# sehyun03/MulActSeg

Measured on AMD Instinct MI355X. Metric: superpixels scored/sec, higher is better.
Workload: dtype f32; 1 GPU; acquisition-round: PixBal+ban-ignore scorer on resident logits, Cityscapes pool shape [4,20,1024,2048] per step; per rank K single-pass scans (class prior + region sums + histograms) of its shard, then exchange 1 (all-gather class sums) + device class weights (k_class_weight) + weighted finalize + ban + exchange 2 (all-gather scores) + replicated K4 (keys, radix sort, fair-counting budget walk) ov; nseg=2048, id_dtype=int64, regions_scored=679936, budget_clicks=11159, regions_selected=6688

## Files before the change

### include/mulactseg_hip.h

```cpp
#ifndef MULACTSEG_HIP_H
#define MULACTSEG_HIP_H

#include <stddef.h>
#include <stdint.h>

#ifdef __cplusplus
extern "C" {
#endif

#define MAS_ID_I64 0
#define MAS_ID_I32 1
#define MAS_ID_U16 2
#define MAS_MAP_U8 3

#define MAS_MAX_CLASSES 32

#define MAS_SCORE_FRAC_BITS 40
#define MAS_PROB_FRAC_BITS 23
#define MAS_LOSS_FRAC_BITS 32

#define MAS_ABI_VERSION 9
int mas_abi_version(void);
const char* mas_error_string(int code);

// ... 62 lines not shown
                               const void* work, const float* grad, const float* weights, int N, int C, int H, int W, int S, float invT,
                               int flags, float* dz, int64_t* dzq_fix, void* stream);


int mas_region_keys(const float* score, const uint8_t* valid, const int32_t* img_rank, int64_t n_img, int S,
                    uint64_t* keys , void* stream);

size_t mas_select_workspace_bytes(int64_t n);

int mas_sort_keys_desc(const uint64_t* keys_in, int64_t n, uint64_t* keys_out, void* workspace, size_t ws_bytes,
                       void* stream);

int mas_budget_walk(const uint64_t* sorted_keys, int64_t n, const uint8_t* region_cost, const int32_t* img_of_rank,
                    int S, int64_t budget, int64_t max_out, int64_t* n_selected,
                    int32_t* sel_img, int32_t* sel_id, float* sel_score, void* workspace, size_t ws_bytes, void* stream);

int mas_region_reweight(float* score, const int32_t* dominant, int64_t n, int ban_class, const float* cls_w ,
                        void* stream);

int mas_dominant_hist(const int32_t* dominant, int64_t n, int C, uint64_t* counts , void* stream);

int mas_minmax_normalize(float* scores, int64_t n, uint32_t* scratch2, void* stream);


#define MAS_LABELS_BAD_VALUE 1

int mas_region_label_counts(const void* spx, int spx_dtype, const uint8_t* labels, int H, int W, int nseg, int num_classes, int trim_k,
                            int32_t* full , int32_t* trimmed , int32_t* status ,
                            void* stream);

// ... 204 lines not shown
```

### mulactseg_amd/_lib.py

```python
import ctypes
import os

_HERE = os.path.dirname(os.path.abspath(__file__))
LIB_PATH = os.environ.get("MAS_LIB") or os.path.join(_HERE, "libmulactseg_hip.so")

ID_I64, ID_I32, ID_U16 = 0, 1, 2
MAP_U8 = 3
MAX_CLASSES = 32
LABELS_BAD_VALUE = 1
SCORE_FRAC, PROB_FRAC, LOSS_FRAC = 40, 23, 32
LOSS_CE, LOSS_GROUP, LOSS_GROUP_ONLY_MULTI, LOSS_DECOMP, LOSS_TCE = 1, 2, 4, 8, 16
ACC_WORDS = 8
GRAD_FRAC = 44
MS_MAX_SOURCES = 16

SK_DMA, SK_NOSPLIT = 1, 2
LOWRES_GENERIC = 1
ABI_VERSION = 9

_c = ctypes
_vp, _i, _f, _i64, _d = _c.c_void_p, _c.c_int, _c.c_float, _c.c_int64, _c.c_double


class SkOpts(ctypes.Structure):
    _fields_ = [("flags", _c.c_uint), ("spin_limit", _c.c_uint), ("stamps", _c.c_void_p)]


SIGNATURES = {
    "mas_abi_version": (_i, []),
    "mas_error_string": (_c.c_char_p, [_i]),
    "mas_class_prob_sum": (_i, [_vp, _i, _i, _i, _i, _f, _vp, _vp]),
    "mas_bvsb_region_accum": (_i, [_vp, _vp, _i, _vp, _i, _i, _i, _i, _i, _f, _vp, _vp, _vp]),
    "mas_region_finalize": (_i, [_vp, _vp, _i64, _i, _i, _vp, _vp, _vp, _vp, _vp]),
    "mas_region_keys": (_i, [_vp, _vp, _vp, _i64, _i, _vp, _vp]),
    "mas_select_workspace_bytes": (_c.c_size_t, [_i64]),
    "mas_sort_keys_desc": (_i, [_vp, _i64, _vp, _vp, _c.c_size_t, _vp]),
    "mas_budget_walk": (_i, [_vp, _i64, _vp, _vp, _i, _i64, _i64, _vp, _vp, _vp, _vp, _vp, _c.c_size_t, _vp]),
    "mas_region_reweight": (_i, [_vp, _vp, _i64, _i, _vp, _vp]),
    "mas_dominant_hist": (_i, [_vp, _i64, _i, _vp, _vp]),
    "mas_minmax_normalize": (_i, [_vp, _i64, _vp, _vp]),
    "mas_region_label_counts": (_i, [_vp, _i, _vp, _i, _i, _i, _i, _i, _vp, _vp, _vp, _vp]),
    "mas_region_multi_hot": (_i, [_vp, _vp, _vp, _i, _i, _vp, _vp, _vp]),
    "mas_region_dominant": (_i, [_vp, _vp, _vp, _i, _i, _i, _vp, _vp]),
    "mas_region_paint": (_i, [_vp, _i, _vp, _i, _i, _i, _vp, _i, _vp, _vp]),
    "mas_spx_max_onehot": (_i, [_vp, _i, _vp, _i, _i, _i, _i, _i, _vp, _vp, _vp, _vp, _vp]),
    "mas_iou_counts": (_i, [_vp, _vp, _vp, _i64, _i, _i64, _vp, _vp]),
    "mas_logits_iou_counts": (_i, [_vp, _vp, _i, _i, _i, _i, _i, _i64, _vp, _vp]),
    "mas_lowres_iou_counts": (_i, [_vp, _vp, _i, _i, _i, _i, _i, _i, _i, _i64, _vp, _vp]),
    "mas_single_pass_accum": (_i, [_vp, _vp, _i, _i, _i, _i, _i, _i, _f, _vp, _vp, _vp, _vp]),
    "mas_single_pass_accum_lowres": (_i, [_vp, _i, _i, _vp, _i, _i, _i, _i, _i, _i, _f, _vp, _vp, _vp, _vp]),
    "mas_single_pass_accum_lowres_opt": (_i, [_vp, _i, _i, _vp, _i, _i, _i, _i, _i, _i, _f, _vp, _vp, _vp, _c.c_uint, _vp]),
    "mas_class_weight": (_i, [_vp, _i, _i, _i64, _i, _i, _d, _vp, _vp, _vp, _vp]),
# ... 141 lines not shown
```

### mulactseg_amd/active_selection/engine.py

```python
import numpy as np
import torch


class ShardPlan:

    def __init__(self, n_img, batch_size, rank=0, world=1):
        self.n_img, self.batch_size, self.rank, self.world = n_img, batch_size, rank, world
        self.n_batches = (n_img + batch_size - 1) // batch_size
        per = (self.n_batches + world - 1) // world
        self.batch_lo = min(rank * per, self.n_batches)
        self.batch_hi = min((rank + 1) * per, self.n_batches)
        self.img_lo = min(self.batch_lo * batch_size, n_img)
        self.img_hi = min(self.batch_hi * batch_size, n_img)
        self.per_rank_imgs = per * batch_size
        self.batch_of = (np.arange(n_img) // batch_size).astype(np.int32)

    @property
    def local_indices(self):
        return list(range(self.img_lo, self.img_hi))

    @property
    def n_local(self):
        return self.img_hi - self.img_lo

# ... 74 lines not shown
        w31 = None if cls_w is None else getattr(cls_w, '_mas_w31', None)
        if w31 is None:
            w = torch.ones(hist.shape[-1], dtype=torch.float32, device=hist.device) if cls_w is None else cls_w.detach().to(hist.device)
            w31 = (w.double() * 2147483648.0).floor().to(torch.int64).view(torch.int32)[::2].contiguous()
        return self.ops.region_finalize_weighted(class_sum, hist, w31, ban_class, want_hist_i64)

    def minmax_normalize_(self, scores):
        return self.ops.minmax_normalize_(scores)

    def region_reweight_(self, scores, dominant, ban_class, cls_w):
        return self.ops.region_reweight_(scores, dominant, ban_class, cls_w)

    def dominant_hist(self, dominant, C):
        return self.ops.dominant_hist(dominant, C)

    def select(self, scores, valid, img_rank, img_of_rank, region_cost, budget, max_out):
        keys = self.ops.region_keys(scores, valid, img_rank)
        skeys = self.ops.sort_keys_desc(keys)
        nsel, simg, sid, ssc = self.ops.budget_walk(skeys, region_cost, img_of_rank, scores.shape[1], budget, max_out)
        n = int(nsel.item())
        return n, simg[:n].cpu().numpy(), sid[:n].cpu().numpy(), ssc[:n].cpu().numpy()

    def local_head(self, plan, scores, valid, img_rank, max_out):
        lo, hi = plan.img_lo, plan.img_hi
        head = torch.zeros(max_out, dtype=torch.int64, device=scores.device)
        if hi > lo:
            keys = self.ops.region_keys(scores[lo:hi].contiguous(), None if valid is None else valid[lo:hi].contiguous(),
                                        img_rank[lo:hi].contiguous())
            m = min(keys.numel(), max_out)
            head[:m] = self.ops.sort_keys_desc(keys)[:m]
        return head

    def walk_heads(self, heads, region_cost, img_of_rank, S, budget, max_out):
        nsel, simg, sid, ssc = self.ops.budget_walk(self.ops.sort_keys_desc(heads), region_cost, img_of_rank, S, budget, max_out)
        n = int(nsel.item())
        return n, simg[:n].cpu().numpy(), sid[:n].cpu().numpy(), ssc[:n].cpu().numpy()

    def select_sharded(self, plan, scores, valid, img_rank, img_of_rank, region_cost, budget, max_out):
        head = self.local_head(plan, scores, valid, img_rank, max_out)
        merged = torch.empty(plan.world * max_out, dtype=torch.int64, device=scores.device)
        _dist().all_gather_into_tensor(merged, head)
        return self.walk_heads(merged, region_cost, img_of_rank, scores.shape[1], budget, max_out)


def default_backend(device):
    return HipBackend(device)


def select_regions(backend, plan, scores, valid, img_rank, img_of_rank, region_cost, budget, max_out):
    if plan.world > 1 and max_out is not None and _dist() is not None and hasattr(backend, 'select_sharded'):
        return backend.select_sharded(plan, scores, valid, img_rank, img_of_rank, region_cost, budget, max_out)
# ... 105 lines not shown
```

### mulactseg_amd/csrc/select.hip

```cpp
#include <cstring>

#include <rocprim/device/device_radix_sort.hpp>
#include <rocprim/device/device_scan.hpp>

#include "common.h"

namespace {

constexpr int kThreads = 256;

__device__ __forceinline__ unsigned order_bits(float f) {
    const unsigned b = mas_f2u(f);
    return (b & 0x80000000u) ? ~b : (b | 0x80000000u);
}
__device__ __forceinline__ float unorder_bits(unsigned o) {
    return mas_u2f((o & 0x80000000u) ? (o & 0x7fffffffu) : ~o);
}

inline int id_bits_for(int S) {
    int b = 1;
    while ((1LL << b) < S) ++b;
    return b;
}

__global__ __launch_bounds__(kThreads) void k_region_keys(const float* __restrict__ score, const unsigned char* __restrict__ valid,
                                                           const int* __restrict__ img_rank, long long n, int S, int id_bits,
                                                           mas_u64* __restrict__ keys) {
    const long long i = (long long)blockIdx.x * kThreads + threadIdx.x;
    if (i >= n) return;
    const long long img = i / S;
    const int id = (int)(i - img * S);
    mas_u64 k = 0;
    if (!valid || valid[i]) {
        const unsigned lo = ((unsigned)img_rank[img] << id_bits) | (unsigned)id;
        k = ((mas_u64)order_bits(score[i]) << 32) | lo;
    }
    keys[i] = k;
}

__global__ __launch_bounds__(kThreads) void k_walk_cost(const mas_u64* __restrict__ keys, long long n,
                                                         const unsigned char* __restrict__ region_cost,
                                                         const int* __restrict__ img_of_rank, int S, int id_bits,
                                                         unsigned* __restrict__ cost) {
    const long long i = (long long)blockIdx.x * kThreads + threadIdx.x;
    if (i >= n) return;
    const mas_u64 k = keys[i];
    unsigned c = 0;
    if (k) {
        c = 1;
        if (region_cost) {
            const unsigned lo = (unsigned)k;
            const int id = (int)(lo & ((1u << id_bits) - 1u));
            const int img = img_of_rank[lo >> id_bits];
            c = (unsigned)region_cost[(long long)img * S + id];
        }
    }
    cost[i] = c;
}

__global__ __launch_bounds__(kThreads) void k_walk_find(const mas_u64* __restrict__ keys, const unsigned* __restrict__ prefix,
                                                         long long n, unsigned long long budget,
                                                         unsigned long long* __restrict__ n_selected) {
    const long long i = (long long)blockIdx.x * kThreads + threadIdx.x;
    if (i >= n) return;
    const bool valid = keys[i] != 0;
    const bool prev_valid = (i == 0) ? true : (keys[i - 1] != 0);
    const bool crossed = valid && (unsigned long long)prefix[i] > budget;
    const bool prev_crossed = (i > 0) && ((unsigned long long)prefix[i - 1] > budget);
    if (crossed && !prev_crossed) atomicMin(n_selected, (unsigned long long)(i + 1));
    if (!valid && prev_valid) atomicMin(n_selected, (unsigned long long)i);
    if (i == n - 1 && valid) atomicMin(n_selected, (unsigned long long)n);
}

__global__ __launch_bounds__(kThreads) void k_walk_emit(const mas_u64* __restrict__ keys, const unsigned long long* __restrict__ n_selected,
                                                         long long max_out, const int* __restrict__ img_of_rank, int id_bits,
                                                         int* __restrict__ sel_img, int* __restrict__ sel_id,
                                                         float* __restrict__ sel_score) {
    const long long i = (long long)blockIdx.x * kThreads + threadIdx.x;
    if (i >= max_out) return;
    int img = -1, id = -1;
    float s = 0.0f;
    if ((unsigned long long)i < *n_selected) {
        const mas_u64 k = keys[i];
        const unsigned lo = (unsigned)k;
        id = (int)(lo & ((1u << id_bits) - 1u));
        img = img_of_rank[lo >> id_bits];
        s = unorder_bits((unsigned)(k >> 32));
    }
    sel_img[i] = img;
    sel_id[i] = id;
    sel_score[i] = s;
}

__global__ void k_set_u64(unsigned long long* p, unsigned long long v) { *p = v; }

__global__ __launch_bounds__(kThreads) void k_region_reweight(float* __restrict__ score, const int* __restrict__ dominant,
                                                               long long n, int ban_class, const float* __restrict__ cls_w) {
    const long long i = (long long)blockIdx.x * kThreads + threadIdx.x;
    if (i >= n) return;
    const int d = dominant[i];
    float s = score[i];
    if (d == ban_class) s = 0.0f;
// ... 60 lines not shown
}

}

extern "C" size_t mas_select_workspace_bytes(int64_t n) {
    if (n <= 0) return 0;
    const size_t t = sort_temp_bytes(n), u = scan_temp_bytes(n);
    return align_up(t > u ? t : u) + 2 * align_up(sizeof(unsigned) * (size_t)n) + 256;
}

extern "C" int mas_region_keys(const float* score, const uint8_t* valid, const int32_t* img_rank, int64_t n_img, int S,
                               uint64_t* keys, void* stream) {
    if (!score || !img_rank || !keys) return MAS_ERR_NULL;
    if (n_img <= 0 || S <= 0) return MAS_ERR_SHAPE;
    const int b = id_bits_for(S);
    if (b > 24 || n_img > (1LL << (32 - b))) return MAS_ERR_RANGE;
    const long long n = (long long)n_img * S;
    const long long nblk = (n + kThreads - 1) / kThreads;
    if (nblk > 0x7fffffffLL) return MAS_ERR_SHAPE;
    hipLaunchKernelGGL(k_region_keys, dim3((unsigned)nblk), dim3(kThreads), 0, static_cast<hipStream_t>(stream), score, valid,
                       img_rank, n, S, b, reinterpret_cast<mas_u64*>(keys));
    return mas_launch_status();
}

extern "C" int mas_sort_keys_desc(const uint64_t* keys_in, int64_t n, uint64_t* keys_out, void* workspace, size_t ws_bytes,
                                  void* stream) {
    if (!keys_in || !keys_out || !workspace) return MAS_ERR_NULL;
    if (n <= 0) return MAS_ERR_SHAPE;
    size_t need = sort_temp_bytes(n);
    if (ws_bytes < need) return MAS_ERR_WORKSPACE;
    hipError_t e = rocprim::radix_sort_keys_desc(workspace, need, reinterpret_cast<const mas_u64*>(keys_in),
// ... 66 lines not shown
```

### mulactseg_amd/csrc/single_pass.hip

```cpp
#include <cstdlib>
#include "common.h"

namespace {

constexpr int kThreads = 256;
constexpr int kTileW = 256;
constexpr int kTileH = 16;
constexpr int kLogSlots = 7;
constexpr int kSlots = 1 << kLogSlots;

__device__ __forceinline__ int table_slot(int* keys, int id) {
    unsigned h = ((unsigned)id * 2654435769u) >> (32 - kLogSlots);
    for (int probe = 0; probe < kSlots; ++probe) {
        int k = __hip_atomic_load(&keys[h], __ATOMIC_RELAXED, __HIP_MEMORY_SCOPE_WORKGROUP);
        if (k == id) return (int)h;
        if (k == -1) {
            int old = atomicCAS(&keys[h], -1, id);
            if (old == -1 || old == id) return (int)h;
        }
        h = (h + 1) & (kSlots - 1);
    }
    return -1;
}

// ... 466 lines not shown
        if (a) atomicAdd(&prob_sum[(size_t)b * C + threadIdx.x], a);
    }
    for (int i = threadIdx.x; i < kSlots * C; i += kThreads) {
        const unsigned n = t_hist[i];
        if (n) {
            const int s = i / C;
            const size_t g = (size_t)t_keys[s] * C + (i - s * C);
            atomicAdd(&ghist[g], n);
            atomicAdd(&gsum[g], t_sum[i]);
        }
    }
}

__global__ __launch_bounds__(kThreads) void k_region_finalize_weighted(const mas_u64* __restrict__ class_sum,
                                                                        const unsigned* __restrict__ hist, long long n_regions,
                                                                        int C, const unsigned* __restrict__ w31, int ban_class,
                                                                        float* __restrict__ score, int* __restrict__ dominant,
                                                                        unsigned* __restrict__ count,
                                                                        long long* __restrict__ hist_i64) {
    extern __shared__ __attribute__((aligned(16))) unsigned char smem[];
    const int CP = C | 1;
    mas_u64* s_sum = reinterpret_cast<mas_u64*>(smem);
    unsigned* s_hist = reinterpret_cast<unsigned*>(s_sum + (size_t)kThreads * CP);
    const long long r0 = (long long)blockIdx.x * kThreads;
    const long long rows = (n_regions - r0) < kThreads ? (n_regions - r0) : kThreads;
    const long long words = rows * C;
    for (long long i = threadIdx.x; i < words; i += kThreads) {
        const int row = (int)(i / C), col = (int)(i - (long long)row * C);
        const unsigned hv = hist[r0 * C + i];
        s_sum[row * CP + col] = class_sum[r0 * C + i];
        s_hist[row * CP + col] = hv;
        if (hist_i64) hist_i64[r0 * C + i] = (long long)hv;
    }
    __syncthreads();
    if ((long long)threadIdx.x >= rows) return;
    const long long r = r0 + threadIdx.x;
    const unsigned* h = s_hist + threadIdx.x * CP;
    const mas_u64* cs = s_sum + threadIdx.x * CP;
    unsigned long long n = 0;
    unsigned best = 0;
    int arg = 0;
    uint64_t hi = 0, lo = 0;
    for (int c = 0; c < C; ++c) {
        const unsigned v = h[c];
        n += v;
        if (v > best) { best = v; arg = c; }
        if (v) mas_mac_u64_u32((uint64_t)cs[c], w31[c], &hi, &lo);
    }
    float sc = 0.0f;
    if (n) sc = mas_fixed_mean(mas_shr31_u128(hi, lo), n, MAS_SCORE_FRAC);
    if (ban_class >= 0 && arg == ban_class) sc = 0.0f;
    score[r] = sc;
    if (dominant) dominant[r] = arg;
    if (count) count[r] = (unsigned)n;
}

inline bool mas_ring_enabled() {
    static const bool on = [] { const char* e = getenv("MAS_SINGLE_PASS_RING"); return !(e && e[0] == '0'); }();
    return on;
}

inline size_t smem_bytes(int C, int CT) {
    return sizeof(mas_u64) * ((size_t)kSlots * C + 4 * CT) + sizeof(unsigned) * (size_t)kSlots * C + sizeof(int) * kSlots;
}

template <int CT, bool EXACT, typename IdT>
int launch(const float* z, const void* spx, int B, int C, int H, int W, int S, float invT, mas_u64* prob_sum, mas_u64* class_sum,
           unsigned* hist, hipStream_t st) {
    const int tiles_x = (W + kTileW - 1) / kTileW;
// ... 125 lines not shown

extern "C" int mas_single_pass_accum_lowres(const float* zq, int h, int w, const void* spx, int spx_dtype, int B, int C, int H, int W, int S,
                                            float invT, uint64_t* prob_sum, uint64_t* class_sum, uint32_t* hist, void* stream) {
    return mas_single_pass_accum_lowres_opt(zq, h, w, spx, spx_dtype, B, C, H, W, S, invT, prob_sum, class_sum, hist, 0u, stream);
}

extern "C" int mas_region_finalize_weighted(const uint64_t* class_sum, const uint32_t* hist, int64_t n_regions, int C,
                                            const uint32_t* w31, int ban_class, float* score, int32_t* dominant, uint32_t* count,
                                            int64_t* hist_i64, void* stream) {
    if (!class_sum || !hist || !w31 || !score) return MAS_ERR_NULL;
    if (n_regions <= 0) return MAS_ERR_SHAPE;
    if (C < 1 || C > MAS_MAX_CLASSES) return MAS_ERR_CLASSES;
    const long long nblk = (n_regions + kThreads - 1) / kThreads;
    if (nblk > 0x7fffffffLL) return MAS_ERR_SHAPE;
    const size_t smem = (sizeof(mas_u64) + sizeof(unsigned)) * (size_t)kThreads * (C | 1);
    hipLaunchKernelGGL(k_region_finalize_weighted, dim3((unsigned)nblk), dim3(kThreads), smem, static_cast<hipStream_t>(stream),
                       reinterpret_cast<const mas_u64*>(class_sum), hist, (long long)n_regions, C, w31, ban_class, score, dominant,
                       count, reinterpret_cast<long long*>(hist_i64));
    return mas_launch_status();
}
```

### mulactseg_amd/ops.py

```python
import ctypes
import os

import numpy as np
import torch

from . import _lib

_ID_CODES = {torch.int64: _lib.ID_I64, torch.int32: _lib.ID_I32, torch.uint16: _lib.ID_U16,
             torch.int16: _lib.ID_U16}


def inv_temperature(T):
    return float(np.float32(1.0) / np.float32(T))


def _stream(t):
    return torch.cuda.current_stream(t.device).cuda_stream


def _need(t, name, dtype=None):
    if not t.is_cuda:
        raise _lib.MulActSegHipError("%s must live on the GPU (no CPU path exists)" % name)
    if dtype is not None and t.dtype != dtype:
        raise TypeError("%s must be %s, got %s" % (name, dtype, t.dtype))
# ... 290 lines not shown
    n = sorted_keys.numel()
    max_out = n if max_out is None else min(n, max_out)
    dev = sorted_keys.device
    lib = _lib.load()
    ws = torch.empty(lib.mas_select_workspace_bytes(n), dtype=torch.uint8, device=dev)
    nsel = torch.empty(1, dtype=torch.int64, device=dev)
    sel_img = torch.empty(max_out, dtype=torch.int32, device=dev)
    sel_id = torch.empty(max_out, dtype=torch.int32, device=dev)
    sel_score = torch.empty(max_out, dtype=torch.float32, device=dev)
    with torch.cuda.device(dev):
        _lib.check(lib.mas_budget_walk(sorted_keys.data_ptr(), n, cost_bits.data_ptr() if cost_bits is not None else None,
                                       img_of_rank.data_ptr(), S, int(budget), max_out, nsel.data_ptr(), sel_img.data_ptr(),
                                       sel_id.data_ptr(), sel_score.data_ptr(), ws.data_ptr(), ws.numel(), _stream(sorted_keys)),
                   "mas_budget_walk")
    return nsel, sel_img, sel_id, sel_score


def minmax_normalize_(scores):
    _need(scores, "scores", torch.float32)
    scratch = torch.empty(2, dtype=torch.int32, device=scores.device)
    with torch.cuda.device(scores.device):
        _lib.check(_lib.load().mas_minmax_normalize(scores.data_ptr(), scores.numel(), scratch.data_ptr(), _stream(scores)),
                   "mas_minmax_normalize")
    return scores


def iou_counts(outputs, outputs_all, targets, num_classes, ignore_label, counts=None):
    _need(targets, "targets", torch.int64)
    if outputs is not None:
        _need(outputs, "outputs", torch.int64)
# ... 1897 lines not shown
```

Baseline: 55.91 million superpixels/s.

## Replace full radix sort with radix-select top-K prefix for budget selection

Adds a multi-pass histogram radix-select that finds the key threshold for the top-K regions and sorts only a small candidate set (up to 4096), instead of building keys for all regions and radix-sorting them before the budget walk. It is used for the single-device select, for the sharded local head and for the head walk, with a fallback to the full sort when the candidate capacity is exceeded or the walk cannot be proven. The finalize-weighted kernel also gets vectorized staging loads and a reciprocal multiply in place of the division by C. The risk is extra kernel passes, plus a host status check that can trigger the fallback path.

```diff
diff --git a/include/mulactseg_hip.h b/include/mulactseg_hip.h
--- a/include/mulactseg_hip.h
+++ b/include/mulactseg_hip.h
@@ -100,6 +100,20 @@
 int mas_budget_walk(const uint64_t* sorted_keys, int64_t n, const uint8_t* region_cost, const int32_t* img_of_rank,
                     int S, int64_t budget, int64_t max_out, int64_t* n_selected,
                     int32_t* sel_img, int32_t* sel_id, float* sel_score, void* workspace, size_t ws_bytes, void* stream);
+
+#define MAS_SELECT_PROVEN 0
+#define MAS_SELECT_CAPACITY 1
+#define MAS_SELECT_OPEN_WALK 2
+size_t mas_select_prefix_workspace_bytes(void);
+int mas_select_prefix_capacity(void);
+
+int mas_select_prefix(const float* score , const uint8_t* valid , const int32_t* img_rank,
+                      const int32_t* img_of_rank, const uint8_t* region_cost , int64_t n_img, int S,
+                      int64_t budget, int64_t K, int32_t* packed, void* workspace, size_t ws_bytes, void* stream);
+int mas_select_prefix_keys(const uint64_t* keys, int64_t n, const int32_t* img_of_rank, const uint8_t* region_cost, int S,
+                           int64_t budget, int64_t K, int32_t* packed, void* workspace, size_t ws_bytes, void* stream);
+int mas_select_head(const float* score, const uint8_t* valid, const int32_t* img_rank, int64_t n_img, int S, int64_t K,
+                    uint64_t* head, int32_t* status, void* workspace, size_t ws_bytes, void* stream);
 
 int mas_region_reweight(float* score, const int32_t* dominant, int64_t n, int ban_class, const float* cls_w ,
                         void* stream);
diff --git a/mulactseg_amd/_lib.py b/mulactseg_amd/_lib.py
--- a/mulactseg_amd/_lib.py
+++ b/mulactseg_amd/_lib.py
@@ -12,6 +12,7 @@
 LOSS_CE, LOSS_GROUP, LOSS_GROUP_ONLY_MULTI, LOSS_DECOMP, LOSS_TCE = 1, 2, 4, 8, 16
 ACC_WORDS = 8
 GRAD_FRAC = 44
+SELECT_PROVEN, SELECT_CAPACITY, SELECT_OPEN_WALK = 0, 1, 2
 MS_MAX_SOURCES = 16
 
 SK_DMA, SK_NOSPLIT = 1, 2
@@ -36,6 +37,11 @@
     "mas_select_workspace_bytes": (_c.c_size_t, [_i64]),
     "mas_sort_keys_desc": (_i, [_vp, _i64, _vp, _vp, _c.c_size_t, _vp]),
     "mas_budget_walk": (_i, [_vp, _i64, _vp, _vp, _i, _i64, _i64, _vp, _vp, _vp, _vp, _vp, _c.c_size_t, _vp]),
+    "mas_select_prefix_workspace_bytes": (_c.c_size_t, []),
+    "mas_select_prefix_capacity": (_i, []),
+    "mas_select_prefix": (_i, [_vp, _vp, _vp, _vp, _vp, _i64, _i, _i64, _i64, _vp, _vp, _c.c_size_t, _vp]),
+    "mas_select_prefix_keys": (_i, [_vp, _i64, _vp, _vp, _i, _i64, _i64, _vp, _vp, _c.c_size_t, _vp]),
+    "mas_select_head": (_i, [_vp, _vp, _vp, _i64, _i, _i64, _vp, _vp, _vp, _c.c_size_t, _vp]),
     "mas_region_reweight": (_i, [_vp, _vp, _i64, _i, _vp, _vp]),
     "mas_dominant_hist": (_i, [_vp, _i64, _i, _vp, _vp]),
     "mas_minmax_normalize": (_i, [_vp, _i64, _vp, _vp]),
diff --git a/mulactseg_amd/active_selection/engine.py b/mulactseg_amd/active_selection/engine.py
--- a/mulactseg_amd/active_selection/engine.py
+++ b/mulactseg_amd/active_selection/engine.py
@@ -112,27 +112,48 @@
     def dominant_hist(self, dominant, C):
         return self.ops.dominant_hist(dominant, C)
 
-    def select(self, scores, valid, img_rank, img_of_rank, region_cost, budget, max_out):
+    def _select_sorted(self, scores, valid, img_rank, img_of_rank, region_cost, budget, max_out):
         keys = self.ops.region_keys(scores, valid, img_rank)
-        skeys = self.ops.sort_keys_desc(keys)
-        nsel, simg, sid, ssc = self.ops.budget_walk(skeys, region_cost, img_of_rank, scores.shape[1], budget, max_out)
+        return self._walk_sorted(self.ops.sort_keys_desc(keys), region_cost, img_of_rank, scores.shape[1], budget, max_out)
+
+    def _walk_sorted(self, skeys, region_cost, img_of_rank, S, budget, max_out):
+        nsel, simg, sid, ssc = self.ops.budget_walk(skeys, region_cost, img_of_rank, S, budget, max_out)
         n = int(nsel.item())
         return n, simg[:n].cpu().numpy(), sid[:n].cpu().numpy(), ssc[:n].cpu().numpy()
 
+    def _proven(self, packed, max_out):
+        status, n, simg, sid, ssc = self.ops.unpack_selection(packed.cpu().numpy(), max_out)
+        self.last_select_status = status
+        return None if status else (n, simg, sid, ssc)
+
+    def select(self, scores, valid, img_rank, img_of_rank, region_cost, budget, max_out):
+        if max_out is not None and 0 < max_out <= self.ops.select_prefix_capacity():
+            max_out = min(int(max_out), scores.numel())
+            got = self._proven(self.ops.select_prefix(scores, valid, img_rank, img_of_rank, region_cost, budget, max_out), max_out)
+            if got is not None:
+                return got
+        return self._select_sorted(scores, valid, img_rank, img_of_rank, region_cost, budget, max_out)
+
     def local_head(self, plan, scores, valid, img_rank, max_out):
         lo, hi = plan.img_lo, plan.img_hi
+        if hi <= lo:
+            return torch.zeros(max_out, dtype=torch.int64, device=scores.device)
+        rows = (scores[lo:hi].contiguous(), None if valid is None else valid[lo:hi].contiguous(), img_rank[lo:hi].contiguous())
+        if max_out <= self.ops.select_prefix_capacity():
+            return self.ops.select_head(*rows, max_out)[0]
         head = torch.zeros(max_out, dtype=torch.int64, device=scores.device)
-        if hi > lo:
-            keys = self.ops.region_keys(scores[lo:hi].contiguous(), None if valid is None else valid[lo:hi].contiguous(),
-                                        img_rank[lo:hi].contiguous())
-            m = min(keys.numel(), max_out)
-            head[:m] = self.ops.sort_keys_desc(keys)[:m]
+        keys = self.ops.region_keys(*rows)
+        m = min(keys.numel(), max_out)
+        head[:m] = self.ops.sort_keys_desc(keys)[:m]
         return head
 
     def walk_heads(self, heads, region_cost, img_of_rank, S, budget, max_out):
-        nsel, simg, sid, ssc = self.ops.budget_walk(self.ops.sort_keys_desc(heads), region_cost, img_of_rank, S, budget, max_out)
-        n = int(nsel.item())
-        return n, simg[:n].cpu().numpy(), sid[:n].cpu().numpy(), ssc[:n].cpu().numpy()
+        if 0 < max_out <= self.ops.select_prefix_capacity():
+            max_out = min(int(max_out), heads.numel())
+            got = self._proven(self.ops.select_prefix_keys(heads, region_cost, img_of_rank, S, budget, max_out), max_out)
+            if got is not None:
+                return got
+        return self._walk_sorted(self.ops.sort_keys_desc(heads), region_cost, img_of_rank, S, budget, max_out)
 
     def select_sharded(self, plan, scores, valid, img_rank, img_of_rank, region_cost, budget, max_out):
         head = self.local_head(plan, scores, valid, img_rank, max_out)
diff --git a/mulactseg_amd/csrc/select.hip b/mulactseg_amd/csrc/select.hip
--- a/mulactseg_amd/csrc/select.hip
+++ b/mulactseg_amd/csrc/select.hip
@@ -4,24 +4,15 @@
 #include <rocprim/device/device_scan.hpp>
 
 #include "common.h"
+#include "select_keys.h"
 
 namespace {
 
 constexpr int kThreads = 256;
 
-__device__ __forceinline__ unsigned order_bits(float f) {
-    const unsigned b = mas_f2u(f);
-    return (b & 0x80000000u) ? ~b : (b | 0x80000000u);
-}
-__device__ __forceinline__ float unorder_bits(unsigned o) {
-    return mas_u2f((o & 0x80000000u) ? (o & 0x7fffffffu) : ~o);
-}
-
-inline int id_bits_for(int S) {
-    int b = 1;
-    while ((1LL << b) < S) ++b;
-    return b;
-}
+__device__ __forceinline__ unsigned order_bits(float f) { return mas_order_bits(f); }
+__device__ __forceinline__ float unorder_bits(unsigned o) { return mas_unorder_bits(o); }
+inline int id_bits_for(int S) { return mas_key_id_bits(S); }
 
 __global__ __launch_bounds__(kThreads) void k_region_keys(const float* __restrict__ score, const unsigned char* __restrict__ valid,
                                                            const int* __restrict__ img_rank, long long n, int S, int id_bits,
@@ -32,8 +23,7 @@
     const int id = (int)(i - img * S);
     mas_u64 k = 0;
     if (!valid || valid[i]) {
-        const unsigned lo = ((unsigned)img_rank[img] << id_bits) | (unsigned)id;
-        k = ((mas_u64)order_bits(score[i]) << 32) | lo;
+        k = mas_key_make(score[i], img_rank[img], id, id_bits);
     }
     keys[i] = k;
 }
@@ -45,17 +35,7 @@
     const long long i = (long long)blockIdx.x * kThreads + threadIdx.x;
     if (i >= n) return;
     const mas_u64 k = keys[i];
-    unsigned c = 0;
-    if (k) {
-        c = 1;
-        if (region_cost) {
-            const unsigned lo = (unsigned)k;
-            const int id = (int)(lo & ((1u << id_bits) - 1u));
-            const int img = img_of_rank[lo >> id_bits];
-            c = (unsigned)region_cost[(long long)img * S + id];
-        }
-    }
-    cost[i] = c;
+    cost[i] = mas_key_cost(k, region_cost, img_of_rank, S, id_bits);
 }
 
 __global__ __launch_bounds__(kThreads) void k_walk_find(const mas_u64* __restrict__ keys, const unsigned* __restrict__ prefix,
@@ -82,10 +62,9 @@
     float s = 0.0f;
     if ((unsigned long long)i < *n_selected) {
         const mas_u64 k = keys[i];
-        const unsigned lo = (unsigned)k;
-        id = (int)(lo & ((1u << id_bits) - 1u));
-        img = img_of_rank[lo >> id_bits];
-        s = unorder_bits((unsigned)(k >> 32));
+        id = mas_key_id(k, id_bits);
+        img = img_of_rank[mas_key_rank(k, id_bits)];
+        s = mas_key_score(k);
     }
     sel_img[i] = img;
     sel_id[i] = id;
@@ -176,7 +155,7 @@
     if (!score || !img_rank || !keys) return MAS_ERR_NULL;
     if (n_img <= 0 || S <= 0) return MAS_ERR_SHAPE;
     const int b = id_bits_for(S);
-    if (b > 24 || n_img > (1LL << (32 - b))) return MAS_ERR_RANGE;
+    if (!mas_key_fits(n_img, S)) return MAS_ERR_RANGE;
     const long long n = (long long)n_img * S;
     const long long nblk = (n + kThreads - 1) / kThreads;
     if (nblk > 0x7fffffffLL) return MAS_ERR_SHAPE;
diff --git a/mulactseg_amd/csrc/select_keys.h b/mulactseg_amd/csrc/select_keys.h
--- /dev/null
+++ b/mulactseg_amd/csrc/select_keys.h
@@ -0,0 +1,34 @@
+#pragma once
+#include "common.h"
+
+__host__ __device__ __forceinline__ unsigned mas_key_order_bits(unsigned b) {
+    return (b & 0x80000000u) ? ~b : (b | 0x80000000u);
+}
+__device__ __forceinline__ unsigned mas_order_bits(float f) { return mas_key_order_bits(mas_f2u(f)); }
+__device__ __forceinline__ unsigned mas_unorder_word(unsigned o) { return (o & 0x80000000u) ? (o & 0x7fffffffu) : ~o; }
+__device__ __forceinline__ float mas_unorder_bits(unsigned o) { return mas_u2f(mas_unorder_word(o)); }
+
+static inline int mas_key_id_bits(int S) {
+    int b = 1;
+    while ((1LL << b) < S) ++b;
+    return b;
+}
+static inline bool mas_key_fits(long long n_img, int S) {
+    const int b = mas_key_id_bits(S);
+    return b <= 24 && n_img <= (1LL << (32 - b));
+}
+
+__device__ __forceinline__ unsigned mas_key_low(int rank, int id, int id_bits) { return ((unsigned)rank << id_bits) | (unsigned)id; }
+__device__ __forceinline__ mas_u64 mas_key_make(float score, int rank, int id, int id_bits) {
+    return ((mas_u64)mas_order_bits(score) << 32) | mas_key_low(rank, id, id_bits);
+}
+__device__ __forceinline__ int mas_key_id(mas_u64 k, int id_bits) { return (int)((unsigned)k & ((1u << id_bits) - 1u)); }
+__device__ __forceinline__ int mas_key_rank(mas_u64 k, int id_bits) { return (int)((unsigned)k >> id_bits); }
+__device__ __forceinline__ unsigned mas_key_score_word(mas_u64 k) { return mas_unorder_word((unsigned)(k >> 32)); }
+__device__ __forceinline__ float mas_key_score(mas_u64 k) { return mas_u2f(mas_key_score_word(k)); }
+__device__ __forceinline__ unsigned mas_key_cost(mas_u64 k, const unsigned char* __restrict__ region_cost,
+                                                 const int* __restrict__ img_of_rank, int S, int id_bits) {
+    if (!k) return 0u;
+    if (!region_cost) return 1u;
+    return (unsigned)region_cost[(long long)img_of_rank[mas_key_rank(k, id_bits)] * S + mas_key_id(k, id_bits)];
+}
diff --git a/mulactseg_amd/csrc/select_prefix.hip b/mulactseg_amd/csrc/select_prefix.hip
--- /dev/null
+++ b/mulactseg_amd/csrc/select_prefix.hip
@@ -0,0 +1,375 @@
+#include "common.h"
+#include "select_keys.h"
+
+namespace {
+
+constexpr int kThreads = 256;
+constexpr int kBins = 2048;
+constexpr int kPasses = 6;
+constexpr int kShift[kPasses] = {53, 42, 32, 21, 10, 0};
+constexpr unsigned kMask[kPasses] = {2047u, 2047u, 1023u, 2047u, 2047u, 1023u};
+constexpr int kCap = 4096;
+constexpr int kSortThreads = 1024;
+constexpr int kItems = 4;
+constexpr int kMaxBlocks = 2048;
+
+struct SelState {
+    mas_u64 lo_key;
+    unsigned above;
+    unsigned bin;
+    unsigned done;
+    unsigned nvalid;
+    unsigned pad[2];
+};
+static_assert(sizeof(SelState) == 32, "SelState is 32 bytes in the workspace");
+
+constexpr size_t kHistBytes = sizeof(unsigned) * kPasses * kBins;
+constexpr size_t kStateOff = kHistBytes;
+constexpr size_t kCountOff = kStateOff + sizeof(SelState) * kPasses;
+constexpr size_t kZeroBytes = kCountOff + 16;
+constexpr size_t kCandOff = kZeroBytes;
+constexpr size_t kWsBytes = kCandOff + sizeof(mas_u64) * kCap;
+static_assert(kZeroBytes % 16 == 0 && kCandOff % 16 == 0, "the zeroed block is a multiple of 16 bytes");
+
+struct FromScores {
+    const float* __restrict__ score;
+    const unsigned char* __restrict__ valid;
+    const int* __restrict__ img_rank;
+    unsigned S;
+    int id_bits;
+    __device__ __forceinline__ bool hi(unsigned i, unsigned* h) const {
+        if (valid && !valid[i]) return false;
+        *h = mas_order_bits(score[i]);
+        return true;
+    }
+    __device__ __forceinline__ unsigned lo(unsigned i) const {
+        const unsigned img = i / S;
+        return mas_key_low(img_rank[img], (int)(i - img * S), id_bits);
+    }
+};
+struct FromKeys {
+    const mas_u64* __restrict__ keys;
+    __device__ __forceinline__ bool hi(unsigned i, unsigned* h) const {
+        const mas_u64 k = keys[i];
+        *h = (unsigned)(k >> 32);
+        return k != 0;
+    }
+    __device__ __forceinline__ unsigned lo(unsigned i) const { return (unsigned)keys[i]; }
+};
+
+template <int p>
+__device__ SelState pick_state(const unsigned* __restrict__ hist_p, SelState prev, unsigned K, unsigned* s_scan) {
+    if (p > 0 && prev.done) return prev;
+    constexpr int kPer = kBins / kThreads;
+    constexpr int kWaves = kThreads / MAS_WAVE;
+    const int t = threadIdx.x, lane = t & (MAS_WAVE - 1), wave = t / MAS_WAVE;
+    unsigned v[kPer], tsum = 0;
+#pragma unroll
+    for (int j = 0; j < kPer; ++j) {
+        v[j] = hist_p[kBins - 1 - (t * kPer + j)];
+        tsum += v[j];
+    }
+    unsigned incl = tsum;
+#pragma unroll
+    for (int off = 1; off < MAS_WAVE; off <<= 1) {
+        const unsigned o = __shfl_up(incl, off, MAS_WAVE);
+        if (lane >= off) incl += o;
+    }
+    __syncthreads();
+    if (lane == MAS_WAVE - 1) s_scan[wave] = incl;
+    if (t == 0) s_scan[kWaves] = 0xffffffffu;
+    __syncthreads();
+    unsigned before = 0, total = 0;
+#pragma unroll
+    for (int w = 0; w < kWaves; ++w) {
+        const unsigned s = s_scan[w];
+        if (w < wave) before += s;
+        total += s;
+    }
+    const unsigned want = K - prev.above;
+    unsigned run = before + incl - tsum;
+#pragma unroll
+    for (int j = 0; j < kPer; ++j) {
+        if (run < want && run + v[j] >= want) {
+            s_scan[kWaves] = (unsigned)(kBins - 1 - (t * kPer + j));
+            s_scan[kWaves + 1] = run;
+            s_scan[kWaves + 2] = v[j];
+        }
+        run += v[j];
+    }
+    __syncthreads();
+    SelState st = prev;
+    if (p == 0) st.nvalid = total;
+    const unsigned d = s_scan[kWaves];
+    if (d == 0xffffffffu && p == 0) {
+        st.lo_key = 1;
+        st.above = 0;
+        st.bin = total;
+    } else if (d == 0xffffffffu) {
+        st.above = (unsigned)kCap + 1u;
+    } else {
+        st.lo_key = prev.lo_key | ((mas_u64)d << kShift[p]);
+        st.above = prev.above + s_scan[kWaves + 1];
+        st.bin = s_scan[kWaves + 2];
+    }
+    st.done = (st.above + st.bin <= (unsigned)kCap) ? 1u : 0u;
+    return st;
+}
+
+__device__ __forceinline__ SelState load_state(const SelState* __restrict__ states, int p) {
+    if (p < 0) return SelState{0, 0, 0, 0, 0, {0, 0}};
+    return states[p];
+}
+
+template <typename Src, int P>
+__global__ __launch_bounds__(kThreads) void k_select_hist(Src src, unsigned n, unsigned K, unsigned char* __restrict__ ws) {
+    __shared__ unsigned s_hist[kBins];
+    __shared__ unsigned s_scan[kThreads / MAS_WAVE + 4];
+    unsigned* hist = reinterpret_cast<unsigned*>(ws);
+    SelState* states = reinterpret_cast<SelState*>(ws + kStateOff);
+    SelState st = SelState{0, 0, 0, 0, 0, {0, 0}};
+    if constexpr (P > 0) {
+        st = pick_state<(P > 0 ? P - 1 : 0)>(hist + (P - 1) * kBins, load_state(states, P - 2), K, s_scan);
+        if (blockIdx.x == 0 && threadIdx.x == 0) states[P - 1] = st;
+        if (st.done) return;
+    }
+    for (int b = threadIdx.x; b < kBins; b += kThreads) s_hist[b] = 0;
+    __syncthreads();
+    const unsigned lo_hi = (unsigned)(st.lo_key >> 32);
+    for (unsigned i = blockIdx.x * kThreads + threadIdx.x; i < n; i += gridDim.x * kThreads) {
+        unsigned h;
+        if (!src.hi(i, &h)) continue;
+        if constexpr (P < 3) {
+            if constexpr (P > 0)
+                if ((h >> (kShift[P > 0 ? P - 1 : 0] - 32)) != (lo_hi >> (kShift[P > 0 ? P - 1 : 0] - 32))) continue;
+            atomicAdd(&s_hist[(h >> (kShift[P] - 32)) & kMask[P]], 1u);
+        } else {
+            if (h != lo_hi) continue;
+            const unsigned l = src.lo(i);
+            if constexpr (P > 3)
+                if ((l >> kShift[P - 1]) != ((unsigned)st.lo_key >> kShift[P - 1])) continue;
+            atomicAdd(&s_hist[(l >> kShift[P]) & kMask[P]], 1u);
+        }
+    }
+    __syncthreads();
+    for (int b = threadIdx.x; b < kBins; b += kThreads) {
+        const unsigned c = s_hist[b];
+        if (c) atomicAdd(&hist[P * kBins + b], c);
+    }
+}
+
+template <typename Src>
+__global__ __launch_bounds__(kThreads) void k_select_compact(Src src, unsigned n, unsigned K, unsigned char* __restrict__ ws) {
+    __shared__ unsigned s_scan[kThreads / MAS_WAVE + 4];
+    unsigned* hist = reinterpret_cast<unsigned*>(ws);
+    SelState* states = reinterpret_cast<SelState*>(ws + kStateOff);
+    unsigned* cand_count = reinterpret_cast<unsigned*>(ws + kCountOff);
+    mas_u64* cand = reinterpret_cast<mas_u64*>(ws + kCandOff);
+    const SelState st = pick_state<kPasses - 1>(hist + (kPasses - 1) * kBins, load_state(states, kPasses - 2), K, s_scan);
+    if (blockIdx.x == 0 && threadIdx.x == 0) states[kPasses - 1] = st;
+    if (!st.done) return;
+    const unsigned lo_hi = (unsigned)(st.lo_key >> 32);
+    for (unsigned i = blockIdx.x * kThreads + threadIdx.x; i < n; i += gridDim.x * kThreads) {
+        unsigned h;
+        if (!src.hi(i, &h) || h < lo_hi) continue;
+        const mas_u64 k = ((mas_u64)h << 32) | src.lo(i);
+        if (k == 0 || k < st.lo_key) continue;
+        const unsigned pos = atomicAdd(cand_count, 1u);
+        if (pos < (unsigned)kCap) cand[pos] = k;
+    }
+}
+
+__global__ __launch_bounds__(kSortThreads) void k_select_finish(const unsigned char* __restrict__ ws, const mas_u64* __restrict__ direct,
+                                                                 int n_direct, int force_status, int mode,
+                                                                 const unsigned char* __restrict__ region_cost,
+                                                                 const int* __restrict__ img_of_rank, int S, int id_bits,
+                                                                 unsigned long long budget, int K, int* __restrict__ packed,
+                                                                 mas_u64* __restrict__ head, int* __restrict__ head_status) {
+    __shared__ mas_u64 s_key[kCap];
+    __shared__ unsigned s_pre[kCap];
+    __shared__ unsigned s_wave[kSortThreads / MAS_WAVE];
+    __shared__ unsigned s_first[2];
+    const int t = threadIdx.x;
+    int status = force_status, m = 0;
+    unsigned nvalid = 0;
+    if (!status) {
+        if (direct) {
+            m = n_direct;
+        } else {
+            const SelState st = reinterpret_cast<const SelState*>(ws + kStateOff)[kPasses - 1];
+            const unsigned cnt = *reinterpret_cast<const unsigned*>(ws + kCountOff);
+            nvalid = st.nvalid;
+            if (!st.done || cnt > (unsigned)kCap) status = MAS_SELECT_CAPACITY;
+            else m = (int)cnt;
+        }
+    }
+    int P = 1;
+    while (P < m) P <<= 1;
+    const mas_u64* src = direct ? direct : reinterpret_cast<const mas_u64*>(ws + kCandOff);
+    for (int i = t; i < kCap; i += kSortThreads) s_key[i] = i < m ? src[i] : 0;
+    if (t == 0) { s_first[0] = (unsigned)kCap; s_first[1] = (unsigned)kCap; }
+    __syncthreads();
+    for (int k = 2; k <= P; k <<= 1) {
+        for (int j = k >> 1; j > 0; j >>= 1) {
+            for (int q = t; q < (P >> 1); q += kSortThreads) {
+                const int i = ((q & ~(j - 1)) << 1) | (q & (j - 1)), l = i | j;
+                const mas_u64 a = s_key[i], b = s_key[l];
+                const bool desc = (i & k) == 0;
+                if (desc ? (a < b) : (a > b)) { s_key[i] = b; s_key[l] = a; }
+            }
+            __syncthreads();
+        }
+    }
+    if (mode == 1) {
+        for (int i = t; i < K; i += kSortThreads) head[i] = (!status && i < P) ? s_key[i] : 0;
+        if (t == 0) *head_status = status;
+        return;
+    }
+    constexpr int kPer = kCap / kSortThreads;
+    const int lane = t & (MAS_WAVE - 1), wave = t / MAS_WAVE;
+    unsigned c[kPer], tsum = 0;
+#pragma unroll
+    for (int j = 0; j < kPer; ++j) {
+        c[j] = mas_key_cost(s_key[t * kPer + j], region_cost, img_of_rank, S, id_bits);
+        tsum += c[j];
+    }
+    unsigned incl = tsum;
+#pragma unroll
+    for (int off = 1; off < MAS_WAVE; off <<= 1) {
+        const unsigned o = __shfl_up(incl, off, MAS_WAVE);
+        if (lane >= off) incl += o;
+    }
+    if (lane == MAS_WAVE - 1) s_wave[wave] = incl;
+    __syncthreads();
+    unsigned run = incl - tsum;
+    for (int w = 0; w < wave; ++w) run += s_wave[w];
+#pragma unroll
+    for (int j = 0; j < kPer; ++j) {
+        run += c[j];
+        s_pre[t * kPer + j] = run;
+    }
+    __syncthreads();
+    for (int i = t; i < kCap; i += kSortThreads) {
+        const bool valid = s_key[i] != 0;
+        const bool crossed = valid && (unsigned long long)s_pre[i] > budget;
+        const bool prev_crossed = i > 0 && (unsigned long long)s_pre[i - 1] > budget;
+        if (crossed && !prev_crossed) atomicMin(&s_first[0], (unsigned)i);
+        if (!valid && (i == 0 || s_key[i - 1] != 0)) atomicMin(&s_first[1], (unsigned)i);
+    }
+    __syncthreads();
+    const unsigned n_keys = s_first[1];
+    unsigned nsel = 0;
+    if (!status) {
+        if (s_first[0] < (unsigned)kCap) nsel = s_first[0] + 1;
+        else if (direct || n_keys == nvalid) nsel = n_keys;
+        else status = MAS_SELECT_OPEN_WALK;
+    }
+    if (status) nsel = 0;
+    int* sel_img = packed + 2;
+    int* sel_id = sel_img + K;
+    int* sel_bits = sel_id + K;
+    for (int i = t; i < K; i += kSortThreads) {
+        int img = -1, id = -1, bits = 0;
+        if ((unsigned)i < nsel) {
+            const mas_u64 k = s_key[i];
+            id = mas_key_id(k, id_bits);
+            img = img_of_rank[mas_key_rank(k, id_bits)];
+            bits = (int)mas_key_score_word(k);
+        }
+        sel_img[i] = img;
+        sel_id[i] = id;
+        sel_bits[i] = bits;
+    }
+    if (t == 0) {
+        packed[0] = status;
+        packed[1] = (int)nsel;
+    }
+}
+
+int scan_blocks(long long n) {
+    const long long b = (n + (long long)kThreads * kItems - 1) / ((long long)kThreads * kItems);
+    return (int)(b < 1 ? 1 : (b > kMaxBlocks ? kMaxBlocks : b));
+}
+
+template <typename Src>
+int launch_select(const Src& src, long long n, long long K, unsigned char* ws, hipStream_t st) {
+    if (hipError_t e = hipMemsetAsync(ws, 0, kZeroBytes, st); e != hipSuccess) return (int)e;
+    const dim3 grid((unsigned)scan_blocks(n)), block(kThreads);
+    const unsigned un = (unsigned)n, uk = (unsigned)K;
+    hipLaunchKernelGGL((k_select_hist<Src, 0>), grid, block, 0, st, src, un, uk, ws);
+    hipLaunchKernelGGL((k_select_hist<Src, 1>), grid, block, 0, st, src, un, uk, ws);
+    hipLaunchKernelGGL((k_select_hist<Src, 2>), grid, block, 0, st, src, un, uk, ws);
+    hipLaunchKernelGGL((k_select_hist<Src, 3>), grid, block, 0, st, src, un, uk, ws);
+    hipLaunchKernelGGL((k_select_hist<Src, 4>), grid, block, 0, st, src, un, uk, ws);
+    hipLaunchKernelGGL((k_select_hist<Src, 5>), grid, block, 0, st, src, un, uk, ws);
+    hipLaunchKernelGGL((k_select_compact<Src>), grid, block, 0, st, src, un, uk, ws);
+    return mas_launch_status();
+}
+
+bool workspace_ok(const void* ws, size_t ws_bytes) { return ws_bytes >= kWsBytes && ((uintptr_t)ws & 15) == 0; }
+
+}
+
+extern "C" size_t mas_select_prefix_workspace_bytes(void) { return kWsBytes; }
+extern "C" int mas_select_prefix_capacity(void) { return kCap; }
+
+extern "C" int mas_select_prefix(const float* score, const uint8_t* valid, const int32_t* img_rank, const int32_t* img_of_rank,
+                                 const uint8_t* region_cost, int64_t n_img, int S, int64_t budget, int64_t K, int32_t* packed,
+                                 void* workspace, size_t ws_bytes, void* stream) {
+    if (!score || !img_rank || !img_of_rank || !packed || !workspace) return MAS_ERR_NULL;
+    if (n_img <= 0 || S <= 0 || K <= 0 || budget < 0) return MAS_ERR_SHAPE;
+    if (!mas_key_fits(n_img, S) || (long long)n_img * S > (1LL << 30) || K > (1LL << 24)) return MAS_ERR_RANGE;
+    if (!workspace_ok(workspace, ws_bytes)) return MAS_ERR_WORKSPACE;
+    hipStream_t st = static_cast<hipStream_t>(stream);
+    unsigned char* ws = static_cast<unsigned char*>(workspace);
+    const int b = mas_key_id_bits(S);
+    const int force = K > kCap ? MAS_SELECT_CAPACITY : 0;
+    if (!force) {
+        const FromScores src{score, valid, img_rank, (unsigned)S, b};
+        if (const int e = launch_select(src, (long long)n_img * S, K, ws, st)) return e;
+    }
+    hipLaunchKernelGGL(k_select_finish, dim3(1), dim3(kSortThreads), 0, st, ws, (const mas_u64*)nullptr, 0, force, 0, region_cost,
+                       img_of_rank, S, b, (unsigned long long)budget, (int)K, packed, (mas_u64*)nullptr, (int*)nullptr);
+    return mas_launch_status();
+}
+
+extern "C" int mas_select_prefix_keys(const uint64_t* keys, int64_t n, const int32_t* img_of_rank, const uint8_t* region_cost, int S,
+                                      int64_t budget, int64_t K, int32_t* packed, void* workspace, size_t ws_bytes, void* stream) {
+    if (!keys || !img_of_rank || !packed || !workspace) return MAS_ERR_NULL;
+    if (n <= 0 || S <= 0 || K <= 0 || budget < 0) return MAS_ERR_SHAPE;
+    if (mas_key_id_bits(S) > 24 || n > (1LL << 30) || K > (1LL << 24)) return MAS_ERR_RANGE;
+    if (!workspace_ok(workspace, ws_bytes)) return MAS_ERR_WORKSPACE;
+    hipStream_t st = static_cast<hipStream_t>(stream);
+    unsigned char* ws = static_cast<unsigned char*>(workspace);
+    const mas_u64* k = reinterpret_cast<const mas_u64*>(keys);
+    const int force = K > kCap ? MAS_SELECT_CAPACITY : 0;
+    const bool direct = n <= kCap;
+    if (!force && !direct) {
+        const FromKeys src{k};
+        if (const int e = launch_select(src, n, K, ws, st)) return e;
+    }
+    hipLaunchKernelGGL(k_select_finish, dim3(1), dim3(kSortThreads), 0, st, ws, direct ? k : (const mas_u64*)nullptr, direct ? (int)n : 0,
+                       force, 0, region_cost, img_of_rank, S, mas_key_id_bits(S), (unsigned long long)budget, (int)K, packed,
+                       (mas_u64*)nullptr, (int*)nullptr);
+    return mas_launch_status();
+}
+
+extern "C" int mas_select_head(const float* score, const uint8_t* valid, const int32_t* img_rank, int64_t n_img, int S, int64_t K,
+                               uint64_t* head, int32_t* status, void* workspace, size_t ws_bytes, void* stream) {
+    if (!score || !img_rank || !head || !status || !workspace) return MAS_ERR_NULL;
+    if (n_img <= 0 || S <= 0 || K <= 0) return MAS_ERR_SHAPE;
+    if (mas_key_id_bits(S) > 24 || (long long)n_img * S > (1LL << 30) || K > (1LL << 24)) return MAS_ERR_RANGE;
+    if (!workspace_ok(workspace, ws_bytes)) return MAS_ERR_WORKSPACE;
+    hipStream_t st = static_cast<hipStream_t>(stream);
+    unsigned char* ws = static_cast<unsigned char*>(workspace);
+    const int b = mas_key_id_bits(S);
+    const int force = K > kCap ? MAS_SELECT_CAPACITY : 0;
+    if (!force) {
+        const FromScores src{score, valid, img_rank, (unsigned)S, b};
+        if (const int e = launch_select(src, (long long)n_img * S, K, ws, st)) return e;
+    }
+    hipLaunchKernelGGL(k_select_finish, dim3(1), dim3(kSortThreads), 0, st, ws, (const mas_u64*)nullptr, 0, force, 1,
+                       (const unsigned char*)nullptr, (const int*)nullptr, S, b, 0ULL, (int)K, (int*)nullptr,
+                       reinterpret_cast<mas_u64*>(head), status);
+    return mas_launch_status();
+}
diff --git a/mulactseg_amd/csrc/single_pass.hip b/mulactseg_amd/csrc/single_pass.hip
--- a/mulactseg_amd/csrc/single_pass.hip
+++ b/mulactseg_amd/csrc/single_pass.hip
@@ -504,8 +504,8 @@
 
 __global__ __launch_bounds__(kThreads) void k_region_finalize_weighted(const mas_u64* __restrict__ class_sum,
                                                                         const unsigned* __restrict__ hist, long long n_regions,
-                                                                        int C, const unsigned* __restrict__ w31, int ban_class,
-                                                                        float* __restrict__ score, int* __restrict__ dominant,
+                                                                        int C, unsigned rcpC, const unsigned* __restrict__ w31,
+                                                                        int ban_class, float* __restrict__ score, int* __restrict__ dominant,
                                                                         unsigned* __restrict__ count,
                                                                         long long* __restrict__ hist_i64) {
     extern __shared__ __attribute__((aligned(16))) unsigned char smem[];
@@ -513,17 +513,74 @@
     mas_u64* s_sum = reinterpret_cast<mas_u64*>(smem);
     unsigned* s_hist = reinterpret_cast<unsigned*>(s_sum + (size_t)kThreads * CP);
     const long long r0 = (long long)blockIdx.x * kThreads;
-    const long long rows = (n_regions - r0) < kThreads ? (n_regions - r0) : kThreads;
-    const long long words = rows * C;
-    for (long long i = threadIdx.x; i < words; i += kThreads) {
-        const int row = (int)(i / C), col = (int)(i - (long long)row * C);
-        const unsigned hv = hist[r0 * C + i];
-        s_sum[row * CP + col] = class_sum[r0 * C + i];
-        s_hist[row * CP + col] = hv;
-        if (hist_i64) hist_i64[r0 * C + i] = (long long)hv;
+    const int rows = (int)((n_regions - r0) < kThreads ? (n_regions - r0) : kThreads);
+    const int words = rows * C;
+    const unsigned* __restrict__ gh = hist + r0 * C;
+    const mas_u64* __restrict__ gs = class_sum + r0 * C;
+    long long* __restrict__ g64 = hist_i64 ? hist_i64 + r0 * C : nullptr;
+    const bool vec = (((uintptr_t)gh | (uintptr_t)gs | (uintptr_t)g64) & 15) == 0;
+    constexpr int kStageBatch = 2;
+    typedef unsigned v4u __attribute__((ext_vector_type(4)));
+    typedef mas_u64 v2q __attribute__((ext_vector_type(2)));
+    typedef long long v2l __attribute__((ext_vector_type(2)));
+    int done = 0;
+    if (vec) {
+        const int groups = words >> 2;
+        done = groups << 2;
+        for (int g0 = threadIdx.x; g0 < groups; g0 += kThreads * kStageBatch) {
+            v4u hv[kStageBatch];
+            v2q sa[kStageBatch], sb[kStageBatch];
+#pragma unroll
+            for (int u = 0; u < kStageBatch; ++u) {
+                const int g = g0 + u * kThreads;
+                if (g < groups) {
+                    hv[u] = *reinterpret_cast<const v4u*>(gh + 4 * g);
+                    sa[u] = *reinterpret_cast<const v2q*>(gs + 4 * g);
+                    sb[u] = *reinterpret_cast<const v2q*>(gs + 4 * g + 2);
+                }
+            }
+#pragma unroll
+            for (int u = 0; u < kStageBatch; ++u) {
+                const int g = g0 + u * kThreads;
+                if (g < groups) {
+                    int row = rcpC ? (int)__umulhi((unsigned)(4 * g), rcpC) : 4 * g, col = 4 * g - row * C;
+                    const mas_u64 sv[4] = {sa[u].x, sa[u].y, sb[u].x, sb[u].y};
+#pragma unroll
+                    for (int k = 0; k < 4; ++k) {
+                        s_sum[row * CP + col] = sv[k];
+                        s_hist[row * CP + col] = hv[u][k];
+                        if (++col == C) { col = 0; ++row; }
+                    }
+                    if (g64) {
+                        *reinterpret_cast<v2l*>(g64 + 4 * g) = (v2l){(long long)hv[u].x, (long long)hv[u].y};
+                        *reinterpret_cast<v2l*>(g64 + 4 * g + 2) = (v2l){(long long)hv[u].z, (long long)hv[u].w};
+                    }
+                }
+            }
+        }
+    }
+    constexpr int kScalarBatch = 4;
+    for (int i0 = done + threadIdx.x; i0 < words; i0 += kThreads * kScalarBatch) {
+        unsigned hv[kScalarBatch];
+        mas_u64 sv[kScalarBatch];
+#pragma unroll
+        for (int u = 0; u < kScalarBatch; ++u) {
+            const int i = i0 + u * kThreads;
+            if (i < words) { hv[u] = gh[i]; sv[u] = gs[i]; }
+        }
+#pragma unroll
+        for (int u = 0; u < kScalarBatch; ++u) {
+            const int i = i0 + u * kThreads;
+            if (i < words) {
+                const int row = rcpC ? (int)__umulhi((unsigned)i, rcpC) : i, col = i - row * C;
+                s_sum[row * CP + col] = sv[u];
+                s_hist[row * CP + col] = hv[u];
+                if (g64) g64[i] = (long long)hv[u];
+            }
+        }
     }
     __syncthreads();
-    if ((long long)threadIdx.x >= rows) return;
+    if ((int)threadIdx.x >= rows) return;
     const long long r = r0 + threadIdx.x;
     const unsigned* h = s_hist + threadIdx.x * CP;
     const mas_u64* cs = s_sum + threadIdx.x * CP;
@@ -543,6 +600,19 @@
     score[r] = sc;
     if (dominant) dominant[r] = arg;
     if (count) count[r] = (unsigned)n;
+}
+
+inline bool finalize_rcp(int C, unsigned* out) {
+    static unsigned table[MAS_MAX_CLASSES + 1] = {};
+    if (C < 1 || C > MAS_MAX_CLASSES) return false;
+    if (C > 1 && !table[C]) {
+        const unsigned rcp = (unsigned)((0x100000000ULL + (unsigned)C - 1) / (unsigned)C);
+        for (unsigned i = 0; i < (unsigned)(kThreads * C); ++i)
+            if ((unsigned)(((unsigned long long)i * rcp) >> 32) != i / (unsigned)C) return false;
+        table[C] = rcp;
+    }
+    *out = table[C];
+    return true;
 }
 
 inline bool mas_ring_enabled() {
@@ -698,8 +768,10 @@
     const long long nblk = (n_regions + kThreads - 1) / kThreads;
     if (nblk > 0x7fffffffLL) return MAS_ERR_SHAPE;
     const size_t smem = (sizeof(mas_u64) + sizeof(unsigned)) * (size_t)kThreads * (C | 1);
+    unsigned rcpC = 0;
+    if (!finalize_rcp(C, &rcpC)) return MAS_ERR_CLASSES;
     hipLaunchKernelGGL(k_region_finalize_weighted, dim3((unsigned)nblk), dim3(kThreads), smem, static_cast<hipStream_t>(stream),
-                       reinterpret_cast<const mas_u64*>(class_sum), hist, (long long)n_regions, C, w31, ban_class, score, dominant,
+                       reinterpret_cast<const mas_u64*>(class_sum), hist, (long long)n_regions, C, rcpC, w31, ban_class, score, dominant,
                        count, reinterpret_cast<long long*>(hist_i64));
     return mas_launch_status();
 }
diff --git a/mulactseg_amd/ops.py b/mulactseg_amd/ops.py
--- a/mulactseg_amd/ops.py
+++ b/mulactseg_amd/ops.py
@@ -328,6 +328,83 @@
                                        sel_id.data_ptr(), sel_score.data_ptr(), ws.data_ptr(), ws.numel(), _stream(sorted_keys)),
                    "mas_budget_walk")
     return nsel, sel_img, sel_id, sel_score
+
+
+_SELECT_WS = {}
+
+
+def select_prefix_capacity():
+    return int(_lib.load().mas_select_prefix_capacity())
+
+
+def _select_ws(dev):
+    nbytes = int(_lib.load().mas_select_prefix_workspace_bytes())
+    return _stream_scratch(_SELECT_WS, dev, lambda: torch.empty(nbytes, dtype=torch.uint8, device=dev), nbytes)
+
+
+def unpack_selection(packed_host, max_out):
+    a = np.asarray(packed_host, dtype=np.int32)
+    status, n = int(a[0]), int(a[1])
+    m = min(n, max_out)
+    return (status, n, a[2:2 + m].copy(), a[2 + max_out:2 + max_out + m].copy(),
+            a[2 + 2 * max_out:2 + 2 * max_out + m].copy().view(np.float32))
+
+
+def select_prefix(scores, valid, img_rank, img_of_rank, region_cost, budget, max_out):
+    _need(scores, "scores", torch.float32)
+    _need(img_rank, "img_rank", torch.int32)
+    _need(img_of_rank, "img_of_rank", torch.int32)
+    n_img, S = scores.shape
+    if valid is not None:
+        valid = _mask_u8(valid)
+        if tuple(valid.shape) != (n_img, S):
+            raise ValueError("valid must be [n_img, S]")
+    if region_cost is not None:
+        _need(region_cost, "region_cost", torch.uint8)
+    dev = scores.device
+    lib = _lib.load()
+    packed = torch.empty(2 + 3 * max_out, dtype=torch.int32, device=dev)
+    with torch.cuda.device(dev):
+        ws = _select_ws(dev)
+        _lib.check(lib.mas_select_prefix(scores.data_ptr(), _opt(valid), img_rank.data_ptr(), img_of_rank.data_ptr(),
+                                         _opt(region_cost), n_img, S, int(budget), int(max_out), packed.data_ptr(),
+                                         ws.data_ptr(), ws.numel(), _stream(scores)), "mas_select_prefix")
+    return packed
+
+
+def select_prefix_keys(keys, region_cost, img_of_rank, S, budget, max_out):
+    _need(keys, "keys", torch.int64)
+    _need(img_of_rank, "img_of_rank", torch.int32)
+    if region_cost is not None:
+        _need(region_cost, "region_cost", torch.uint8)
+    dev = keys.device
+    lib = _lib.load()
+    packed = torch.empty(2 + 3 * max_out, dtype=torch.int32, device=dev)
+    with torch.cuda.device(dev):
+        ws = _select_ws(dev)
+        _lib.check(lib.mas_select_prefix_keys(keys.data_ptr(), keys.numel(), img_of_rank.data_ptr(), _opt(region_cost), S, int(budget),
+                                              int(max_out), packed.data_ptr(), ws.data_ptr(), ws.numel(), _stream(keys)),
+                   "mas_select_prefix_keys")
+    return packed
+
+
+def select_head(scores, valid, img_rank, max_out):
+    _need(scores, "scores", torch.float32)
+    _need(img_rank, "img_rank", torch.int32)
+    n_img, S = scores.shape
+    if valid is not None:
+        valid = _mask_u8(valid)
+        if tuple(valid.shape) != (n_img, S):
+            raise ValueError("valid must be [n_img, S]")
+    dev = scores.device
+    lib = _lib.load()
+    head = torch.empty(max_out, dtype=torch.int64, device=dev)
+    status = torch.empty(1, dtype=torch.int32, device=dev)
+    with torch.cuda.device(dev):
+        ws = _select_ws(dev)
+        _lib.check(lib.mas_select_head(scores.data_ptr(), _opt(valid), img_rank.data_ptr(), n_img, S, int(max_out), head.data_ptr(),
+                                       status.data_ptr(), ws.data_ptr(), ws.numel(), _stream(scores)), "mas_select_head")
+    return head, status
 
 
 def minmax_normalize_(scores):
```

Measured after the change: 53.76 million superpixels/s. 3.8% lower.
